# fims9000/SYNT_ISIC

Measured on AMD Instinct MI355X. Metric: images/sec at 3x64x64 T=1000 (DDPM reverse-diffusion sampling), higher is better.
Workload: dtype f32

## Files before the change

synt_isic_amd/csrc/conv_plan.cpp:

```cpp
#include "conv_plan.h"
#include "poison_switch.h"

#include <algorithm>
#include <cstdio>
#include <cstdlib>

namespace sisic {

namespace {

struct Switches { bool wino_wide, wino_bf3, wino_col, ksplit, pointwise, pointwise_bf3, pointwise_ksplit, s2_bf3, pointwise_staged_ksplit; };
const Switches& switches() {
    static const Switches sw{env_on("SISIC_WINO_WIDE"), env_on("SISIC_WINO_BF16X3"), env_on("SISIC_WINO_COL"), env_on("SISIC_KSPLIT"),
                             env_on("SISIC_POINTWISE"), env_on("SISIC_POINTWISE_BF16X3"), env_on("SISIC_POINTWISE_KSPLIT"), env_on("SISIC_S2_BF16X3"),
                             env_on("SISIC_POINTWISE_STAGED_KSPLIT")};
    return sw;
}

}

bool poison_alloc() {
    static const bool on = [] { const char* e = std::getenv("SISIC_POISON_ALLOC"); return e && std::atoi(e) != 0; }();
    return on;
}

namespace {

struct DirectTiling { int cfg, ks, stride, tw, th, wn; };
constexpr DirectTiling DIRECT[] = {
#define X(id, KS, STRIDE, MT, NT, WM, WN, TW, CIC, OCC, KSP) {id, KS, STRIDE, TW, WN * NT * 32 / TW, WN},
// ... 92 lines not shown
    if (a.tile_cfg == CFG_PWB_STAGED_KSPLIT) {
        PLAN_REFUSE_UNLESS((Cin / 8) % (4 * PWB_WAVES) == 0, "conv2d(pointwise bf16x3, staged K-split): tile_cfg 37 needs a multiple of 128 input channels");
        PLAN_REFUSE_UNLESS(HW % 64 == 0, "conv2d(pointwise bf16x3, staged K-split): tile_cfg 37 needs whole 64-pixel tiles");
        PLAN_REFUSE_UNLESS(a.Cout == 64 || a.Cout == 128 || a.Cout == 256, "conv2d(pointwise bf16x3, staged K-split): tile_cfg 37 needs 64, 128 or 256 output channels");
        PLAN_REFUSE_UNLESS(a.gn_scale == nullptr, "conv2d(pointwise bf16x3, staged K-split): tile_cfg 37 has no GroupNorm prologue");
        PLAN_REFUSE_UNLESS(!a.relu, "conv2d(pointwise bf16x3, staged K-split): tile_cfg 37 has no relu");
        PLAN_REFUSE_UNLESS(a.Cout % 64 != 0 || pwbsk_lds_bytes(Cin, a.Cout) <= PWBSK_MAX_LDS, "conv2d(pointwise bf16x3, staged K-split): tile_cfg 37 needs %zu bytes of LDS", pwbsk_lds_bytes(Cin, a.Cout));
    }
    PLAN_REFUSE_UNLESS(conv_pointwise_bf3_applicable(a), "conv2d(pointwise bf16x3): shape not supported by tile_cfg 28");
    const bool ks_ok = (Cin / 8) % (4 * PWB_WAVES) == 0;
    const bool staged_ok = a.Cout / 64 >= 6 && a.Cout / 64 <= PWBS_MAX_WAVES && pwbs_lds_bytes(Cin) <= 150 * 1024;
    if (a.tile_cfg == CFG_PWB_KSPLIT) PLAN_REFUSE_UNLESS(ks_ok, "conv2d(pointwise bf16x3, K-split): tile_cfg 35 needs a multiple of 128 input channels");
    if (a.tile_cfg == CFG_PWB_STAGED) PLAN_REFUSE_UNLESS(staged_ok, "conv2d(pointwise bf16x3, staged): tile_cfg 34 needs 384 .. 768 output channels and at most %d input channels", (150 * 1024) / 392);
    if (a.tile_cfg == CFG_PWB_STAGED_KSPLIT || (a.tile_cfg == 0 && pwbsk_routed(a, ks_ok))) pl.form = PWB_FORM_STAGED_KSPLIT;
    else if (a.tile_cfg == CFG_PWB_KSPLIT || (a.tile_cfg == 0 && ks_ok && HW <= 256 && a.Cout <= 256 && switches().pointwise_ksplit)) pl.form = PWB_FORM_KSPLIT;
    else if (a.tile_cfg == CFG_PWB_STAGED || (a.tile_cfg == 0 && staged_ok && (int64_t)a.B * (HW / 64) >= 128)) pl.form = PWB_FORM_STAGED;
    else if (a.tile_cfg == CFG_PWB_64PX || (a.tile_cfg != CFG_PWB_32PX && (int64_t)a.B * (HW / 64) * (a.Cout / 64) >= 2048)) pl.form = PWB_FORM_64PX;
    else pl.form = PWB_FORM_32PX;
    pl.carries_rider = a.gn_scale == nullptr && pl.form != PWB_FORM_STAGED;
}

int plan_direct(const sisic_conv_args& a, ConvPlan& pl) {
    const Switches& sw = switches();
    int cfg = a.tile_cfg;
    SISIC_REQUIRE(!wino_cfg_row(cfg), "conv2d: tile_cfg %d needs w_winograd, ksize 3 and stride 1", cfg);
    int Ht = pl.Hout, Wt = pl.Wout;
    if (a.ksize == 7) {
        if (cfg == 0) cfg = 41;
    } else if (a.ksize == 1 && a.stride == 2) {
        if (cfg == 0) cfg = Wt >= 24 ? 31 : (Wt >= 12 ? 32 : 33);
    } else if (a.ksize == 1) {
        SISIC_REQUIRE(!a.upsample, "conv2d: 1x1 with upsample");
        const bool pwb_forced = (cfg >= CFG_PWB && cfg <= CFG_PWB_64PX) || cfg == CFG_PWB_STAGED || cfg == CFG_PWB_KSPLIT || cfg == CFG_PWB_STAGED_KSPLIT;
        if (pwb_forced || (cfg == 0 && sw.pointwise_bf3 && conv_pointwise_bf3_applicable(a))) {
// ... 84 lines not shown
```

synt_isic_amd/csrc/conv_plan.h:

```cpp
#pragma once

#include "common.h"

namespace sisic {

enum ConvCfg : int {
    CFG_AUTO = 0, CFG_POINTWISE = 20, CFG_PWB = 28, CFG_PWB_32PX = 29, CFG_PWB_64PX = 30, CFG_PWB_STAGED = 34, CFG_PWB_KSPLIT = 35,
    CFG_S2_BF3 = 36, CFG_PWB_STAGED_KSPLIT = 37, CFG_SMALL_32ROWS = 50, CFG_SMALL_8ROWS = 51, CFG_SMALL_ONE_GROUP = 52,
    CFG_WINO_1IMG_8W = 60, CFG_WINO_4IMG_8W = 61, CFG_WINO_1IMG_16W = 62, CFG_WINO_4IMG_16W = 63,
    CFG_WINO_1IMG_8W_STAG = 64, CFG_WINO_4IMG_8W_STAG = 65, CFG_WINO_1IMG_16W_STAG = 66, CFG_WINO_4IMG_16W_STAG = 67,
    CFG_WINO_WIDE128 = 68, CFG_WINO_WIDE64 = 69, CFG_WINO_COL128 = 70, CFG_WINO_COL64 = 71, CFG_WINO_SECOND128 = 72, CFG_WINO_SECOND64 = 73,
    CFG_WINO_BF3 = 74, CFG_WINO_LATENCY128 = 78, CFG_WINO_LATENCY64 = 79, CFG_KSPLIT8_FIRST = 90, CFG_KSPLIT8_PAIR = 91, CFG_KSPLIT8_BF3 = 92,
};

#define SISIC_DIRECT_TILINGS(X) \
    X(1, 3, 1, 2, 2, 1, 4, 64, 8, 2, 1)  X(2, 3, 1, 2, 2, 1, 4, 32, 8, 2, 1)  X(3, 3, 1, 2, 2, 1, 4, 16, 8, 2, 1) \
    X(4, 3, 1, 1, 1, 2, 2, 8, 8, 2, 1)  X(5, 3, 1, 2, 1, 1, 4, 16, 8, 2, 1)  X(6, 3, 1, 2, 1, 1, 4, 64, 8, 2, 1) \
    X(7, 3, 1, 2, 1, 1, 4, 32, 8, 2, 1)  X(8, 3, 1, 1, 2, 2, 4, 32, 8, 4, 1)  X(9, 3, 1, 1, 2, 2, 4, 16, 8, 4, 1) \
    X(10, 3, 1, 1, 2, 2, 4, 32, 8, 2, 1)  X(14, 3, 1, 1, 1, 2, 4, 16, 8, 4, 1)  X(15, 3, 1, 1, 1, 2, 4, 8, 8, 4, 1) \
    X(16, 3, 1, 1, 1, 2, 2, 8, 16, 2, 2)  X(17, 3, 1, 1, 1, 2, 2, 8, 8, 2, 2)  X(11, 3, 2, 2, 1, 1, 4, 32, 8, 2, 1) \
    X(12, 3, 2, 2, 1, 1, 4, 16, 8, 2, 1)  X(13, 3, 2, 1, 1, 2, 2, 8, 8, 2, 1)  X(18, 3, 2, 1, 1, 2, 2, 8, 16, 2, 2) \
    X(19, 3, 2, 1, 1, 2, 2, 8, 8, 2, 2)  X(21, 1, 1, 2, 2, 1, 4, 256, 16, 2, 1)  X(22, 1, 1, 1, 1, 2, 2, 64, 16, 2, 1) \
    X(23, 1, 1, 2, 1, 1, 4, 128, 16, 2, 1)  X(24, 1, 1, 1, 2, 2, 4, 256, 32, 4, 1)  X(25, 1, 1, 1, 1, 2, 4, 128, 32, 4, 1) \
    X(26, 1, 1, 1, 2, 2, 4, 256, 16, 4, 1)  X(27, 1, 1, 1, 1, 2, 4, 128, 16, 4, 1)  X(31, 1, 2, 2, 1, 1, 4, 32, 16, 2, 1) \
    X(32, 1, 2, 2, 1, 1, 4, 16, 16, 2, 1)  X(33, 1, 2, 1, 1, 2, 2, 8, 16, 2, 1)  X(41, 7, 2, 2, 1, 1, 4, 32, 2, 2, 1) \
    X(42, 7, 2, 2, 1, 1, 4, 32, 4, 2, 1)

enum ConvKernel { CK_SMALLCOUT, CK_DIRECT, CK_POINTWISE, CK_POINTWISE_BF3, CK_S2_BF3, CK_WINO_FIRST, CK_WINO_SECOND, CK_WINO_THIRD, CK_WINO_BF3 };
enum PwbForm { PWB_FORM_KSPLIT, PWB_FORM_STAGED, PWB_FORM_64PX, PWB_FORM_32PX, PWB_FORM_STAGED_KSPLIT };
enum ReduceForm { REDUCE_ANY, REDUCE_64PX };

enum WinoGeometry { WG_FIRST, WG_SECOND, WG_BF3 };
struct WinoCfg {
    int cfg;
    WinoGeometry geom;
    int imgs, waves;
    bool stagger;
    int col;
    int ksplit;
    int tile_h, tile_w;
    int profile_slot;
};
const WinoCfg* wino_cfg_row(int cfg);

constexpr int CS_TW = 32, CS_CIC = 2;
constexpr int PWB_WAVES = 4;
constexpr int PWBS_MAX_WAVES = 12;
inline size_t pwbs_lds_bytes(int Cin) { return (size_t)(Cin / 8) * 2 * 64 * 24 + 8 * (size_t)Cin; }
constexpr int PWBSK_MAX_WAVES = 16, PWBSK_CAP = 8;
constexpr size_t PWBSK_MAX_LDS = 128 * 1024;
inline size_t pwbsk_lds_bytes(int Cin, int Cout) {
    const int nl = Cin / 8 / PWB_WAVES;
    const size_t operands = (size_t)PWB_WAVES * (nl < PWBSK_CAP ? nl : PWBSK_CAP) * 2 * 64 * 24, partials = (size_t)PWB_WAVES * (Cout / 64) * 32 * 64 * 4;
    return operands > partials ? operands : partials;
}

struct ConvPlan {
    ConvKernel kernel;
    int cfg;
    int form;
    int Hout, Wout, stats_slots;
    bool finalizes, carries_rider;
    int ksplit;
// ... 11 lines not shown
```

synt_isic_amd/csrc/conv_pointwise_bf3.hip:

```cpp
#include <cstdlib>
#include <type_traits>

#include "conv_plan.h"
#include "gn_finalize.h"

namespace sisic {

typedef float pwb_f32x16 __attribute__((ext_vector_type(16)));
typedef short pwb_bf16x8 __attribute__((ext_vector_type(8)));
typedef unsigned pwb_u4 __attribute__((ext_vector_type(4)));
typedef unsigned pwb_u2 __attribute__((ext_vector_type(2)));
typedef float pwb_f2 __attribute__((ext_vector_type(2)));
typedef float pwb_f4 __attribute__((ext_vector_type(4)));

struct PwbParams {
    const float* in0;
    const float* in1;
    int c0, c1, B, HW;
    const float* wb;
    int n_co64;
    const float* bias;
    int Cout;
    const float* gn_scale;
    const float* gn_shift;
    const float* chan_bias;
    int chan_bias_stride;
    const float* residual;
    int relu;
    float* out;
    float* stats;
    int n_px, n_co_items, nitems, nwg, nchunks;
    int n_rider_wg;
    GnFinJob rider;
};


__device__ __forceinline__ float pwb_half_wave_sum(float v) {
    v += __int_as_float(__builtin_amdgcn_update_dpp(0, __float_as_int(v), 0xB1, 0xf, 0xf, true));
    v += __int_as_float(__builtin_amdgcn_update_dpp(0, __float_as_int(v), 0x4E, 0xf, 0xf, true));
    v += __int_as_float(__builtin_amdgcn_update_dpp(0, __float_as_int(v), 0x141, 0xf, 0xf, true));
    v += __int_as_float(__builtin_amdgcn_update_dpp(0, __float_as_int(v), 0x140, 0xf, 0xf, true));
    return v + __shfl_xor(v, 16);
}
__device__ __forceinline__ float pwb_row16_sum(float v) {
    v += __int_as_float(__builtin_amdgcn_update_dpp(0, __float_as_int(v), 0xB1, 0xf, 0xf, true));
    v += __int_as_float(__builtin_amdgcn_update_dpp(0, __float_as_int(v), 0x4E, 0xf, 0xf, true));
    v += __int_as_float(__builtin_amdgcn_update_dpp(0, __float_as_int(v), 0x141, 0xf, 0xf, true));
    v += __int_as_float(__builtin_amdgcn_update_dpp(0, __float_as_int(v), 0x140, 0xf, 0xf, true));
// ... 404 lines not shown
        for (int i = 0; i < XD; ++i) {
            if (c + i < nl) {
                const Tup t = make(c + i, xr[i]);
                if (c + i + XD < nl) load_x(cb + c + i + XD, xr[i]);
                if ((i & 1) == 0) {
                    mm(t, ua, ul);
                    if (c + i + 2 < nl) load_f(cb + c + i + 2, ua, ul);
                } else {
                    mm(t, ub, um);
                    if (c + i + 2 < nl) load_f(cb + c + i + 2, ub, um);
                }
            }
        }
    }

#pragma unroll
    for (int x = 0; x < CB; ++x)
#pragma unroll
        for (int r = 0; r < 16; ++r) P_lds[((wave_u * 2 + x) * 16 + r) * 64 + lane] = acc[x][r];
    __syncthreads();
    const int x = wave_u >> 1, rb = 8 * (wave_u & 1);
    const __amdgpu_buffer_rsrc_t rso = __builtin_amdgcn_make_buffer_rsrc(p.out + (size_t)b * p.Cout * HW, 0, -1, 0x00020000);
    const __amdgpu_buffer_rsrc_t rsr = __builtin_amdgcn_make_buffer_rsrc(
        const_cast<float*>(p.residual ? p.residual + (size_t)b * p.Cout * HW : p.out), 0, -1, 0x00020000);
    const unsigned o_voff = 4u * (unsigned)((4 * half) * HW + px0 + l31);
    const int slots = HW / 32;
    float add[8], res[8];
#pragma unroll
    for (int rr = 0; rr < 8; ++rr) {
        const int r = rb + rr;
        const int cs = co0 + 32 * x + 8 * (r >> 2) + (r & 3);
        const int col = cs + 4 * half;
        add[rr] = 0.0f;
        if (p.bias) add[rr] += p.bias[col];
        if (p.chan_bias) add[rr] += p.chan_bias[(size_t)b * p.chan_bias_stride + col];
        res[rr] = 0.0f;
        if (p.residual) res[rr] = __builtin_bit_cast(float, __builtin_amdgcn_raw_buffer_load_b32(rsr, o_voff, 4u * (unsigned)(cs * HW), 0));
    }
#pragma unroll
    for (int rr = 0; rr < 8; ++rr) {
        const int r = rb + rr;
        const int cs = co0 + 32 * x + 8 * (r >> 2) + (r & 3);
        float part[PWB_WAVES];
#pragma unroll
        for (int k = 0; k < PWB_WAVES; ++k) part[k] = P_lds[((k * 2 + x) * 16 + r) * 64 + lane];
        float v = ((part[0] + part[1]) + part[2]) + part[3];
        v = v + add[rr] + res[rr];
        if (p.relu) v = fmaxf(v, 0.0f);
        __builtin_amdgcn_raw_buffer_store_b32(__float_as_uint(v), rso, o_voff, 4u * (unsigned)(cs * HW), 0);
        if (p.stats) {
            const int co = cs + 4 * half;
            const float s1 = pwb_half_wave_sum(v);
            const float d = v - s1 * (1.0f / 32.0f);
            float dd;
            asm volatile("v_mul_f32 %0, %1, %1" : "=v"(dd) : "v"(d));
            const float q = pwb_half_wave_sum(dd);
            if (l31 == 0)
                reinterpret_cast<float4*>(p.stats)[((size_t)b * p.Cout + co) * slots + px_t] = make_float4(32.0f, s1, q, 0.0f);
        }
    }
}

__device__ __forceinline__ void pwbs_load_chunk(const __amdgpu_buffer_rsrc_t rs0, const __amdgpu_buffer_rsrc_t rs1, const int c0, const int HW,
                                                const int c, const unsigned x_voff, pwb_f2 (&xr)[4]) {
    const int cc0 = 8 * c;
    if (cc0 < c0) {
        const unsigned soff = 4u * (unsigned)(cc0 * HW);
#pragma unroll
        for (int k = 0; k < 4; ++k) xr[k] = __builtin_bit_cast(pwb_f2, __builtin_amdgcn_raw_buffer_load_b64(rs0, x_voff, soff + 4u * (unsigned)(k * HW), 0));
    } else {
        const unsigned soff = 4u * (unsigned)((cc0 - c0) * HW);
#pragma unroll
        for (int k = 0; k < 4; ++k) xr[k] = __builtin_bit_cast(pwb_f2, __builtin_amdgcn_raw_buffer_load_b64(rs1, x_voff, soff + 4u * (unsigned)(k * HW), 0));
    }
}
template <int PRO>
__device__ __forceinline__ void pwbs_split_store(const pwb_f2 (&xr)[4], const float* gp, unsigned* const S_hm, unsigned* const S_lo, const int slot,
                                                 const int lane) {
    pwb_f4 g01 = {1.0f, 0.0f, 1.0f, 0.0f}, g23 = g01;
    if constexpr (PRO != 0) {
        g01 = *reinterpret_cast<const pwb_f4*>(gp);
        g23 = *reinterpret_cast<const pwb_f4*>(gp + 4);
    }
#pragma unroll
    for (int nb = 0; nb < 2; ++nb) {
        float v[4];
#pragma unroll
        for (int k = 0; k < 4; ++k) {
            float e = nb ? xr[k].y : xr[k].x;
            if constexpr (PRO != 0) {
                const float sc = k == 0 ? g01.x : (k == 1 ? g01.z : (k == 2 ? g23.x : g23.z));
                const float sh = k == 0 ? g01.y : (k == 1 ? g01.w : (k == 2 ? g23.y : g23.w));
                e = e * sc + sh;
                if constexpr (PRO == 2) e = pwb_silu(e);
            }
            v[k] = e;
        }
        unsigned hi[2], mid[2], lo[2];
#pragma unroll
        for (int q = 0; q < 2; ++q) {
            const float v0 = v[2 * q], v1 = v[2 * q + 1];
            const unsigned h0 = __float_as_uint(v0) & 0xffff0000u, h1 = __float_as_uint(v1) & 0xffff0000u;
            const float r0 = v0 - __uint_as_float(h0), r1 = v1 - __uint_as_float(h1);
            const unsigned m0 = __float_as_uint(r0) & 0xffff0000u, m1 = __float_as_uint(r1) & 0xffff0000u;
            const float l0 = r0 - __uint_as_float(m0), l1 = r1 - __uint_as_float(m1);
            hi[q] = __builtin_amdgcn_perm(h1, h0, 0x07060302u);
            mid[q] = __builtin_amdgcn_perm(m1, m0, 0x07060302u);
            lo[q] = __builtin_amdgcn_perm(__float_as_uint(l1), __float_as_uint(l0), 0x07060302u);
        }
        *reinterpret_cast<pwb_u4*>(S_hm + ((size_t)(slot * 2 + nb) * 64 + lane) * 4) = pwb_u4{hi[0], hi[1], mid[0], mid[1]};
        *reinterpret_cast<pwb_u2*>(S_lo + ((size_t)(slot * 2 + nb) * 64 + lane) * 2) = pwb_u2{lo[0], lo[1]};
    }
}
__device__ __forceinline__ void pwbs_read_b(const unsigned* const S_hm, const unsigned* const S_lo, const int slot, const int nb, const int lane,
                                            pwb_u4& hm, pwb_u4& mh, pwb_u4& lh) {
    hm = *reinterpret_cast<const pwb_u4*>(S_hm + ((size_t)(slot * 2 + nb) * 64 + lane) * 4);
    const pwb_u2 lo = *reinterpret_cast<const pwb_u2*>(S_lo + ((size_t)(slot * 2 + nb) * 64 + lane) * 2);
    mh = pwb_u4{hm.z, hm.w, hm.x, hm.y};
    lh = pwb_u4{lo.x, lo.y, hm.x, hm.y};
}

template <int PRO>
__global__ void __launch_bounds__(64 * PWBS_MAX_WAVES) conv_pwbs_kernel(const PwbParams p) {
    extern __shared__ __attribute__((aligned(16))) float smem[];
    int wg;
    {
        const int L = blockIdx.x, nwg = p.nwg;
        const int xcd = L & 7, slot = L >> 3, q = nwg >> 3, r = nwg & 7;
        wg = (xcd < r ? xcd * (q + 1) : r * (q + 1) + (xcd - r) * q) + slot;
    }
    const int tid = threadIdx.x, lane = tid & 63;
    const int wave_u = __builtin_amdgcn_readfirstlane(tid >> 6);
    const int nwaves = p.n_co_items;
    const int half = lane >> 5, l31 = lane & 31;
    int px_t = wg % p.n_px, b = wg / p.n_px;
    asm volatile("" : "+s"(px_t), "+s"(b));
    constexpr int CB = 2, NB = 2;
    const int co_i = wave_u;
    const int px0 = 64 * px_t, co0 = 64 * co_i;
    const int Cin = p.c0 + p.c1, HW = p.HW, n = p.nchunks;

    const __amdgpu_buffer_rsrc_t rs0 = __builtin_amdgcn_make_buffer_rsrc(const_cast<float*>(p.in0 + (size_t)b * p.c0 * HW), 0, -1, 0x00020000);
    const __amdgpu_buffer_rsrc_t rs1 = __builtin_amdgcn_make_buffer_rsrc(
        const_cast<float*>(p.in1 ? p.in1 + (size_t)b * p.c1 * HW : p.in0), 0, -1, 0x00020000);
    const __amdgpu_buffer_rsrc_t rsw = __builtin_amdgcn_make_buffer_rsrc(const_cast<float*>(p.wb), 0, -1, 0x00020000);
    const unsigned x_voff = 4u * (unsigned)((4 * half) * HW + px0 + NB * l31);
    const unsigned a_lane16 = 16u * (unsigned)lane, a_lane8 = 8u * (unsigned)lane;

    unsigned* const S_hm = reinterpret_cast<unsigned*>(smem);
    unsigned* const S_lo = S_hm + (size_t)n * NB * 64 * 4;
    float* const gnL = reinterpret_cast<float*>(S_lo + (size_t)n * NB * 64 * 2);
    if constexpr (PRO != 0) {
        for (int i = tid; i < Cin; i += 64 * nwaves) {
            gnL[2 * i] = p.gn_scale[(size_t)b * Cin + i];
            gnL[2 * i + 1] = p.gn_shift[(size_t)b * Cin + i];
        }
        __syncthreads();
    }
    for (int c = wave_u; c < n; c += nwaves) {
        pwb_f2 xr[4];
        pwbs_load_chunk(rs0, rs1, p.c0, HW, c, x_voff, xr);
        pwbs_split_store<PRO>(xr, gnL + 2 * (8 * c + 4 * half), S_hm, S_lo, c, lane);
    }
    __syncthreads();

    pwb_f32x16 acc[CB][NB];
#pragma unroll
    for (int x = 0; x < CB; ++x)
#pragma unroll
        for (int nb = 0; nb < NB; ++nb)
#pragma unroll
            for (int r = 0; r < 16; ++r) acc[x][nb][r] = 0.0f;
    pwb_u4 ua[CB], ub[CB];
    pwb_u2 ul[CB], um[CB];
    auto load_f = [&](int c, pwb_u4 (&fa)[CB], pwb_u2 (&fl)[CB]) {
        const unsigned s0 = 3072u * (unsigned)(c * p.n_co64 + co_i);
#pragma unroll
        for (int x = 0; x < CB; ++x) {
            fa[x] = __builtin_amdgcn_raw_buffer_load_b128(rsw, a_lane16, s0 + 1024u * (unsigned)x, 0);
            fl[x] = __builtin_amdgcn_raw_buffer_load_b64(rsw, a_lane8, s0 + 2048u + 512u * (unsigned)x, 0);
        }
    };
    auto chunk = [&](int c, const pwb_u4 (&fa)[CB], const pwb_u2 (&fl)[CB]) {
#pragma unroll
        for (int nb = 0; nb < NB; ++nb) {
            pwb_u4 hm, mh, lh;
            pwbs_read_b(S_hm, S_lo, c, nb, lane, hm, mh, lh);
#pragma unroll
            for (int x = 0; x < CB; ++x) {
                const pwb_u4 a_hl = {fa[x].x, fa[x].y, fl[x].x, fl[x].y};
                acc[x][nb] = __builtin_amdgcn_mfma_f32_32x32x16_bf16(__builtin_bit_cast(pwb_bf16x8, fa[x]), __builtin_bit_cast(pwb_bf16x8, hm), acc[x][nb], 0, 0, 0);
                acc[x][nb] = __builtin_amdgcn_mfma_f32_32x32x16_bf16(__builtin_bit_cast(pwb_bf16x8, fa[x]), __builtin_bit_cast(pwb_bf16x8, mh), acc[x][nb], 0, 0, 0);
                acc[x][nb] = __builtin_amdgcn_mfma_f32_32x32x16_bf16(__builtin_bit_cast(pwb_bf16x8, a_hl), __builtin_bit_cast(pwb_bf16x8, lh), acc[x][nb], 0, 0, 0);
            }
        }
    };
    load_f(0, ua, ul);
    if (n > 1) load_f(1, ub, um);
    {
        int c = 0;
        for (; c + 1 < n; c += 2) {
            chunk(c, ua, ul);
            if (c + 2 < n) load_f(c + 2, ua, ul);
            chunk(c + 1, ub, um);
            if (c + 3 < n) load_f(c + 3, ub, um);
        }
        if (c < n) chunk(c, ua, ul);
    }

    const __amdgpu_buffer_rsrc_t rso = __builtin_amdgcn_make_buffer_rsrc(p.out + (size_t)b * p.Cout * HW, 0, -1, 0x00020000);
    const __amdgpu_buffer_rsrc_t rsr = __builtin_amdgcn_make_buffer_rsrc(
        const_cast<float*>(p.residual ? p.residual + (size_t)b * p.Cout * HW : p.out), 0, -1, 0x00020000);
    const unsigned o_voff = 4u * (unsigned)((4 * half) * HW + px0 + NB * l31);
    const int slots = HW / 32;
#pragma unroll
    for (int x = 0; x < CB; ++x) {
        float add[16];
        pwb_f2 res[16];
#pragma unroll
        for (int r = 0; r < 16; ++r) {
            const int cs = co0 + 32 * x + 8 * (r >> 2) + (r & 3);
            const int col = cs + 4 * half;
            add[r] = 0.0f;
            if (p.bias) add[r] += p.bias[col];
            if (p.chan_bias) add[r] += p.chan_bias[(size_t)b * p.chan_bias_stride + col];
            res[r] = pwb_f2{0.0f, 0.0f};
            if (p.residual) res[r] = __builtin_bit_cast(pwb_f2, __builtin_amdgcn_raw_buffer_load_b64(rsr, o_voff, 4u * (unsigned)(cs * HW), 0));
        }
#pragma unroll
        for (int r = 0; r < 16; ++r) {
            const int cs = co0 + 32 * x + 8 * (r >> 2) + (r & 3);
            float vv[2];
#pragma unroll
            for (int nb = 0; nb < NB; ++nb) {
                vv[nb] = acc[x][nb][r] + add[r] + (nb ? res[r].y : res[r].x);
                if (p.relu) vv[nb] = fmaxf(vv[nb], 0.0f);
            }
            __builtin_amdgcn_raw_buffer_store_b64(pwb_u2{__float_as_uint(vv[0]), __float_as_uint(vv[1])}, rso, o_voff, 4u * (unsigned)(cs * HW), 0);
            if (p.stats) {
                const int co = cs + 4 * half;
                const float s1 = pwb_row16_sum(vv[0] + vv[1]);
                const float mean = s1 * (1.0f / 32.0f);
                const float d0 = vv[0] - mean, d1 = vv[1] - mean;
                float q0, q1;
                asm volatile("v_mul_f32 %0, %2, %2\n\tv_mul_f32 %1, %3, %3" : "=&v"(q0), "=&v"(q1) : "v"(d0), "v"(d1));
                const float q = pwb_row16_sum(q0 + q1);
                if ((l31 & 15) == 0)
                    reinterpret_cast<float4*>(p.stats)[((size_t)b * p.Cout + co) * slots + 2 * px_t + (l31 >> 4)] = make_float4(32.0f, s1, q, 0.0f);
            }
        }
    }
}

#ifndef PWBSK_VAR
#define PWBSK_VAR 0
#endif
__global__ void __launch_bounds__(64 * PWBSK_MAX_WAVES) conv_pwbsk_kernel(const PwbParams p) {
    extern __shared__ __attribute__((aligned(16))) float smem[];
    const int tid = threadIdx.x, lane = tid & 63;
    const int wave_u = __builtin_amdgcn_readfirstlane(tid >> 6);
    const int nwaves = PWB_WAVES * p.n_co_items;
    int L = blockIdx.x;
    if (L < p.n_rider_wg) {
// ... 85 lines not shown
            chunk(kq * cap + j, ua, ul);
            if (p0 + j + 2 < nl) load_f(cb + p0 + j + 2, ua, ul);
            chunk(kq * cap + j + 1, ub, um);
            if (p0 + j + 3 < nl) load_f(cb + p0 + j + 3, ub, um);
        }
#else
        acc[0][0][0] += __uint_as_float(ua[0].x ^ ub[1].y ^ ul[0].x ^ um[1].y) + __uint_as_float(S_hm[lane + 64 * kq]);
#endif
    }

    const __amdgpu_buffer_rsrc_t rso = __builtin_amdgcn_make_buffer_rsrc(p.out + (size_t)b * p.Cout * HW, 0, -1, 0x00020000);
    const __amdgpu_buffer_rsrc_t rsr = __builtin_amdgcn_make_buffer_rsrc(
        const_cast<float*>(p.residual ? p.residual + (size_t)b * p.Cout * HW : p.out), 0, -1, 0x00020000);
    const unsigned o_voff = 4u * (unsigned)((4 * half) * HW + px0 + NB * l31);
    const int slots = HW / 32;
#pragma unroll
    for (int x = 0; x < CB; ++x) {
#if (PWBSK_VAR & 4) == 0
        __syncthreads();
#pragma unroll
        for (int nb = 0; nb < NB; ++nb)
#pragma unroll
            for (int r = 0; r < 16; ++r) P_lds[((wave_u * NB + nb) * 16 + r) * 64 + lane] = acc[x][nb][r];
        __syncthreads();
#endif
        float add[4];
        pwb_f2 res[4];
#pragma unroll
        for (int rr = 0; rr < 4; ++rr) {
            const int cs = co0 + 32 * x + 8 * kq + rr;
            const int col = cs + 4 * half;
            add[rr] = 0.0f;
            if (p.bias) add[rr] += p.bias[col];
            if (p.chan_bias) add[rr] += p.chan_bias[(size_t)b * p.chan_bias_stride + col];
            res[rr] = pwb_f2{0.0f, 0.0f};
            if (p.residual) res[rr] = __builtin_bit_cast(pwb_f2, __builtin_amdgcn_raw_buffer_load_b64(rsr, o_voff, 4u * (unsigned)(cs * HW), 0));
        }
#pragma unroll
        for (int rr = 0; rr < 4; ++rr) {
            const int r = 4 * kq + rr;
            const int cs = co0 + 32 * x + 8 * kq + rr;
            float vv[NB];
#pragma unroll
            for (int nb = 0; nb < NB; ++nb) {
                float part[PWB_WAVES];
#if (PWBSK_VAR & 4) == 0
#pragma unroll
                for (int k = 0; k < PWB_WAVES; ++k) part[k] = P_lds[(((co_i * PWB_WAVES + k) * NB + nb) * 16 + r) * 64 + lane];
#else
#pragma unroll
                for (int k = 0; k < PWB_WAVES; ++k) part[k] = acc[x][nb][4 * k + rr];
#endif
// ... 41 lines not shown
    p.n_px = p.HW / 32;
    const int64_t nitems = (int64_t)p.B * p.n_px * p.n_co_items;
    SISIC_REQUIRE(nitems > 0 && nitems < (int64_t(1) << 31), "conv2d(pointwise bf16x3, K-split): grid too large");
    p.nitems = (int)nitems;
    p.nwg = p.nitems;
    SISIC_REQUIRE((int64_t)p.nwg + p.n_rider_wg < (int64_t(1) << 31), "conv2d(pointwise bf16x3, K-split): grid too large");
    const size_t lds = sizeof(float) * (size_t)(PWB_WAVES * 32 * 64 + (PRO ? 2 * Cin : 0));
    static std::atomic<uint64_t> opt{0};
    auto kern = conv_pwbk_kernel<PRO>;
    SISIC_TRY(ensure_dynamic_lds(ctx, reinterpret_cast<const void*>(kern), (int)lds, opt));
    hipLaunchKernelGGL(kern, dim3(p.n_rider_wg + p.nwg), dim3(64 * PWB_WAVES), lds, s, p);
    SISIC_HIP(hipGetLastError());
    return SISIC_OK;
}

template <int PRO>
static int launch_pwbs(sisic_ctx* ctx, PwbParams& p, int Cin, hipStream_t s) {
    p.n_co_items = p.Cout / 64;
    p.n_px = p.HW / 64;
    const int64_t nwg = (int64_t)p.B * p.n_px;
    SISIC_REQUIRE(nwg > 0 && nwg < (int64_t(1) << 31), "conv2d(pointwise bf16x3, staged): grid too large");
    p.nwg = (int)nwg;
    p.nitems = p.nwg * p.n_co_items;
    const size_t lds = pwbs_lds_bytes(Cin);
    static std::atomic<uint64_t> opt{0};
    auto kern = conv_pwbs_kernel<PRO>;
    SISIC_TRY(ensure_dynamic_lds(ctx, reinterpret_cast<const void*>(kern), (int)lds, opt));
    hipLaunchKernelGGL(kern, dim3(p.nwg), dim3(64 * p.n_co_items), lds, s, p);
    SISIC_HIP(hipGetLastError());
    return SISIC_OK;
}

bool conv_pointwise_bf3_applicable(const sisic_conv_args& a) {
    if (a.ksize != 1 || a.stride != 1 || a.upsample) return false;
    const int HW = a.Hin * a.Win, Cin = a.c0 + a.c1;
    if (HW % 64 != 0 || Cin % 8 != 0 || (a.c1 != 0 && a.c0 % 8 != 0) || a.Cout % 64 != 0) return false;
    if (((reinterpret_cast<uintptr_t>(a.in0) | reinterpret_cast<uintptr_t>(a.in1) | reinterpret_cast<uintptr_t>(a.out) |
          reinterpret_cast<uintptr_t>(a.residual)) & 7) != 0) return false;
    if (4.0 * std::max(std::max(a.c0, a.c1), a.Cout) * HW >= 4294967296.0 || 6.0 * conv_cin_pad(Cin, 1) * conv_cout_pad(a.Cout) >= 4294967296.0) return false;
    if (a.gn_scale && Cin > 1024) return false;
    return true;
}

// ... 15 lines not shown
    return SISIC_OK;
}

int launch_conv_pointwise_bf3(sisic_ctx* ctx, const sisic_conv_args& a, const ConvPlan& plan, hipStream_t s, const GnFinJob* rider) {
    PwbParams p{};
    const int Cin = a.c0 + a.c1;
    p.in0 = a.in0; p.in1 = a.in1; p.c0 = a.c0; p.c1 = a.c1; p.B = a.B; p.HW = a.Hin * a.Win;
    p.wb = a.w_packed + 2 * (size_t)conv_cin_pad(Cin, 1) * conv_cout_pad(a.Cout);
    p.n_co64 = conv_cout_pad(a.Cout) / 64;
    p.bias = a.bias; p.Cout = a.Cout;
    p.gn_scale = a.gn_scale; p.gn_shift = a.gn_shift;
    p.chan_bias = a.chan_bias; p.chan_bias_stride = a.chan_bias_stride; p.residual = a.residual; p.relu = a.relu;
    p.out = a.out; p.stats = a.stats_out;
    p.nchunks = Cin / 8;
    const int pro = a.gn_scale == nullptr ? 0 : (a.gn_silu ? 2 : 1);
    static_assert(PWB_WAVES == GNF_WAVES, "a rider workgroup runs one finalisation job per wave");
    if (rider) { p.rider = *rider; p.n_rider_wg = cdiv(rider->n_jobs, GNF_WAVES); }
    switch (plan.form) {
        case PWB_FORM_STAGED_KSPLIT:
            return launch_pwbsk(ctx, p, Cin, s, rider);
        case PWB_FORM_KSPLIT:
            return pro == 2 ? launch_pwbk<2>(ctx, p, Cin, s) : pro == 1 ? launch_pwbk<1>(ctx, p, Cin, s) : launch_pwbk<0>(ctx, p, Cin, s);
        case PWB_FORM_STAGED:
            return pro == 2 ? launch_pwbs<2>(ctx, p, Cin, s) : pro == 1 ? launch_pwbs<1>(ctx, p, Cin, s) : launch_pwbs<0>(ctx, p, Cin, s);
        case PWB_FORM_64PX:
            return pro == 2 ? launch_pwb<2, 2>(ctx, p, Cin, s) : pro == 1 ? launch_pwb<1, 2>(ctx, p, Cin, s) : launch_pwb<0, 2>(ctx, p, Cin, s);
        default:
            return pro == 2 ? launch_pwb<2, 1>(ctx, p, Cin, s) : pro == 1 ? launch_pwb<1, 1>(ctx, p, Cin, s) : launch_pwb<0, 1>(ctx, p, Cin, s);
    }
}

}
```

Measured before the change: 12.41.

## Add 32-pixel staged pointwise form, deeper weight prefetch, and optional early epilogue loads

Adds a staged pointwise bf16x3 variant that handles 32 pixels per workgroup and splits output channels across two workgroups, meant for 64-pixel feature maps with many output channels. It sits behind an environment switch. The staged kernel now prefetches weight fragments to a configurable depth and overlaps them with the input staging, batching several input chunk loads per wave. An opt-in flag hoists bias and residual loads ahead of the LDS barrier in two epilogues. With default settings only the deeper prefetch, batched staging and hoisted bias path change, at the cost of more register pressure.

```diff
diff --git a/synt_isic_amd/csrc/conv_plan.cpp b/synt_isic_amd/csrc/conv_plan.cpp
--- a/synt_isic_amd/csrc/conv_plan.cpp
+++ b/synt_isic_amd/csrc/conv_plan.cpp
@@ -9,11 +9,11 @@
 
 namespace {
 
-struct Switches { bool wino_wide, wino_bf3, wino_col, ksplit, pointwise, pointwise_bf3, pointwise_ksplit, s2_bf3, pointwise_staged_ksplit; };
+struct Switches { bool wino_wide, wino_bf3, wino_col, ksplit, pointwise, pointwise_bf3, pointwise_ksplit, s2_bf3, pointwise_staged_ksplit, pointwise_staged32; };
 const Switches& switches() {
     static const Switches sw{env_on("SISIC_WINO_WIDE"), env_on("SISIC_WINO_BF16X3"), env_on("SISIC_WINO_COL"), env_on("SISIC_KSPLIT"),
                              env_on("SISIC_POINTWISE"), env_on("SISIC_POINTWISE_BF16X3"), env_on("SISIC_POINTWISE_KSPLIT"), env_on("SISIC_S2_BF16X3"),
-                             env_on("SISIC_POINTWISE_STAGED_KSPLIT")};
+                             env_on("SISIC_POINTWISE_STAGED_KSPLIT"), env_on("SISIC_POINTWISE_STAGED32")};
     return sw;
 }
 
@@ -136,10 +136,12 @@
     if (a.tile_cfg == CFG_PWB_STAGED) PLAN_REFUSE_UNLESS(staged_ok, "conv2d(pointwise bf16x3, staged): tile_cfg 34 needs 384 .. 768 output channels and at most %d input channels", (150 * 1024) / 392);
     if (a.tile_cfg == CFG_PWB_STAGED_KSPLIT || (a.tile_cfg == 0 && pwbsk_routed(a, ks_ok))) pl.form = PWB_FORM_STAGED_KSPLIT;
     else if (a.tile_cfg == CFG_PWB_KSPLIT || (a.tile_cfg == 0 && ks_ok && HW <= 256 && a.Cout <= 256 && switches().pointwise_ksplit)) pl.form = PWB_FORM_KSPLIT;
+    else if (a.tile_cfg == 0 && switches().pointwise_staged32 && HW == 64 && a.Cout >= 384 && a.Cout / 64 <= PWBS_MAX_WAVES && pwbs_lds_bytes(Cin, 1) <= 150 * 1024)
+        pl.form = PWB_FORM_STAGED_32PX;
     else if (a.tile_cfg == CFG_PWB_STAGED || (a.tile_cfg == 0 && staged_ok && (int64_t)a.B * (HW / 64) >= 128)) pl.form = PWB_FORM_STAGED;
     else if (a.tile_cfg == CFG_PWB_64PX || (a.tile_cfg != CFG_PWB_32PX && (int64_t)a.B * (HW / 64) * (a.Cout / 64) >= 2048)) pl.form = PWB_FORM_64PX;
     else pl.form = PWB_FORM_32PX;
-    pl.carries_rider = a.gn_scale == nullptr && pl.form != PWB_FORM_STAGED;
+    pl.carries_rider = a.gn_scale == nullptr && pl.form != PWB_FORM_STAGED && pl.form != PWB_FORM_STAGED_32PX;
 }
 
 int plan_direct(const sisic_conv_args& a, ConvPlan& pl) {
diff --git a/synt_isic_amd/csrc/conv_plan.h b/synt_isic_amd/csrc/conv_plan.h
--- a/synt_isic_amd/csrc/conv_plan.h
+++ b/synt_isic_amd/csrc/conv_plan.h
@@ -27,7 +27,7 @@
     X(42, 7, 2, 2, 1, 1, 4, 32, 4, 2, 1)
 
 enum ConvKernel { CK_SMALLCOUT, CK_DIRECT, CK_POINTWISE, CK_POINTWISE_BF3, CK_S2_BF3, CK_WINO_FIRST, CK_WINO_SECOND, CK_WINO_THIRD, CK_WINO_BF3 };
-enum PwbForm { PWB_FORM_KSPLIT, PWB_FORM_STAGED, PWB_FORM_64PX, PWB_FORM_32PX, PWB_FORM_STAGED_KSPLIT };
+enum PwbForm { PWB_FORM_KSPLIT, PWB_FORM_STAGED, PWB_FORM_64PX, PWB_FORM_32PX, PWB_FORM_STAGED_KSPLIT, PWB_FORM_STAGED_32PX };
 enum ReduceForm { REDUCE_ANY, REDUCE_64PX };
 
 enum WinoGeometry { WG_FIRST, WG_SECOND, WG_BF3 };
@@ -46,7 +46,7 @@
 constexpr int CS_TW = 32, CS_CIC = 2;
 constexpr int PWB_WAVES = 4;
 constexpr int PWBS_MAX_WAVES = 12;
-inline size_t pwbs_lds_bytes(int Cin) { return (size_t)(Cin / 8) * 2 * 64 * 24 + 8 * (size_t)Cin; }
+inline size_t pwbs_lds_bytes(int Cin, int nb = 2) { return (size_t)(Cin / 8) * nb * 64 * 24 + 8 * (size_t)Cin; }
 constexpr int PWBSK_MAX_WAVES = 16, PWBSK_CAP = 8;
 constexpr size_t PWBSK_MAX_LDS = 128 * 1024;
 inline size_t pwbsk_lds_bytes(int Cin, int Cout) {
diff --git a/synt_isic_amd/csrc/conv_pointwise_bf3.hip b/synt_isic_amd/csrc/conv_pointwise_bf3.hip
--- a/synt_isic_amd/csrc/conv_pointwise_bf3.hip
+++ b/synt_isic_amd/csrc/conv_pointwise_bf3.hip
@@ -32,6 +32,8 @@
     int n_px, n_co_items, nitems, nwg, nchunks;
     int n_rider_wg;
     GnFinJob rider;
+    int co_split;
+    int early_epilogue;
 };
 
 
@@ -466,28 +468,37 @@
         }
     }
 
-#pragma unroll
-    for (int x = 0; x < CB; ++x)
-#pragma unroll
-        for (int r = 0; r < 16; ++r) P_lds[((wave_u * 2 + x) * 16 + r) * 64 + lane] = acc[x][r];
-    __syncthreads();
     const int x = wave_u >> 1, rb = 8 * (wave_u & 1);
     const __amdgpu_buffer_rsrc_t rso = __builtin_amdgcn_make_buffer_rsrc(p.out + (size_t)b * p.Cout * HW, 0, -1, 0x00020000);
     const __amdgpu_buffer_rsrc_t rsr = __builtin_amdgcn_make_buffer_rsrc(
         const_cast<float*>(p.residual ? p.residual + (size_t)b * p.Cout * HW : p.out), 0, -1, 0x00020000);
     const unsigned o_voff = 4u * (unsigned)((4 * half) * HW + px0 + l31);
     const int slots = HW / 32;
-    float add[8], res[8];
+    float bv[8], cv[8], res[8], add[8];
+    auto fetch_epilogue = [&]() {
+#pragma unroll
+        for (int rr = 0; rr < 8; ++rr) {
+            const int r = rb + rr;
+            const int cs = co0 + 32 * x + 8 * (r >> 2) + (r & 3);
+            const int col = cs + 4 * half;
+            bv[rr] = cv[rr] = res[rr] = 0.0f;
+            if (p.bias) bv[rr] = p.bias[col];
+            if (p.chan_bias) cv[rr] = p.chan_bias[(size_t)b * p.chan_bias_stride + col];
+            if (p.residual) res[rr] = __builtin_bit_cast(float, __builtin_amdgcn_raw_buffer_load_b32(rsr, o_voff, 4u * (unsigned)(cs * HW), 0));
+        }
+    };
+    if (p.early_epilogue) fetch_epilogue();
+#pragma unroll
+    for (int xx = 0; xx < CB; ++xx)
+#pragma unroll
+        for (int r = 0; r < 16; ++r) P_lds[((wave_u * 2 + xx) * 16 + r) * 64 + lane] = acc[xx][r];
+    __syncthreads();
+    if (!p.early_epilogue) fetch_epilogue();
 #pragma unroll
     for (int rr = 0; rr < 8; ++rr) {
-        const int r = rb + rr;
-        const int cs = co0 + 32 * x + 8 * (r >> 2) + (r & 3);
-        const int col = cs + 4 * half;
         add[rr] = 0.0f;
-        if (p.bias) add[rr] += p.bias[col];
-        if (p.chan_bias) add[rr] += p.chan_bias[(size_t)b * p.chan_bias_stride + col];
-        res[rr] = 0.0f;
-        if (p.residual) res[rr] = __builtin_bit_cast(float, __builtin_amdgcn_raw_buffer_load_b32(rsr, o_voff, 4u * (unsigned)(cs * HW), 0));
+        if (p.bias) add[rr] += bv[rr];
+        if (p.chan_bias) add[rr] += cv[rr];
     }
 #pragma unroll
     for (int rr = 0; rr < 8; ++rr) {
@@ -513,20 +524,26 @@
     }
 }
 
+template <int NB = 2>
+__device__ __forceinline__ pwb_f2 pwbs_load_px(const __amdgpu_buffer_rsrc_t rs, const unsigned voff, const unsigned soff) {
+    if constexpr (NB == 2) return __builtin_bit_cast(pwb_f2, __builtin_amdgcn_raw_buffer_load_b64(rs, voff, soff, 0));
+    else return pwb_f2{__builtin_bit_cast(float, __builtin_amdgcn_raw_buffer_load_b32(rs, voff, soff, 0)), 0.0f};
+}
+template <int NB = 2>
 __device__ __forceinline__ void pwbs_load_chunk(const __amdgpu_buffer_rsrc_t rs0, const __amdgpu_buffer_rsrc_t rs1, const int c0, const int HW,
                                                 const int c, const unsigned x_voff, pwb_f2 (&xr)[4]) {
     const int cc0 = 8 * c;
     if (cc0 < c0) {
         const unsigned soff = 4u * (unsigned)(cc0 * HW);
 #pragma unroll
-        for (int k = 0; k < 4; ++k) xr[k] = __builtin_bit_cast(pwb_f2, __builtin_amdgcn_raw_buffer_load_b64(rs0, x_voff, soff + 4u * (unsigned)(k * HW), 0));
+        for (int k = 0; k < 4; ++k) xr[k] = pwbs_load_px<NB>(rs0, x_voff, soff + 4u * (unsigned)(k * HW));
     } else {
         const unsigned soff = 4u * (unsigned)((cc0 - c0) * HW);
 #pragma unroll
-        for (int k = 0; k < 4; ++k) xr[k] = __builtin_bit_cast(pwb_f2, __builtin_amdgcn_raw_buffer_load_b64(rs1, x_voff, soff + 4u * (unsigned)(k * HW), 0));
-    }
-}
-template <int PRO>
+        for (int k = 0; k < 4; ++k) xr[k] = pwbs_load_px<NB>(rs1, x_voff, soff + 4u * (unsigned)(k * HW));
+    }
+}
+template <int PRO, int NB = 2>
 __device__ __forceinline__ void pwbs_split_store(const pwb_f2 (&xr)[4], const float* gp, unsigned* const S_hm, unsigned* const S_lo, const int slot,
                                                  const int lane) {
     pwb_f4 g01 = {1.0f, 0.0f, 1.0f, 0.0f}, g23 = g01;
@@ -535,7 +552,7 @@
         g23 = *reinterpret_cast<const pwb_f4*>(gp + 4);
     }
 #pragma unroll
-    for (int nb = 0; nb < 2; ++nb) {
+    for (int nb = 0; nb < NB; ++nb) {
         float v[4];
 #pragma unroll
         for (int k = 0; k < 4; ++k) {
@@ -560,19 +577,29 @@
             mid[q] = __builtin_amdgcn_perm(m1, m0, 0x07060302u);
             lo[q] = __builtin_amdgcn_perm(__float_as_uint(l1), __float_as_uint(l0), 0x07060302u);
         }
-        *reinterpret_cast<pwb_u4*>(S_hm + ((size_t)(slot * 2 + nb) * 64 + lane) * 4) = pwb_u4{hi[0], hi[1], mid[0], mid[1]};
-        *reinterpret_cast<pwb_u2*>(S_lo + ((size_t)(slot * 2 + nb) * 64 + lane) * 2) = pwb_u2{lo[0], lo[1]};
-    }
-}
+        *reinterpret_cast<pwb_u4*>(S_hm + ((size_t)(slot * NB + nb) * 64 + lane) * 4) = pwb_u4{hi[0], hi[1], mid[0], mid[1]};
+        *reinterpret_cast<pwb_u2*>(S_lo + ((size_t)(slot * NB + nb) * 64 + lane) * 2) = pwb_u2{lo[0], lo[1]};
+    }
+}
+template <int NB = 2>
 __device__ __forceinline__ void pwbs_read_b(const unsigned* const S_hm, const unsigned* const S_lo, const int slot, const int nb, const int lane,
                                             pwb_u4& hm, pwb_u4& mh, pwb_u4& lh) {
-    hm = *reinterpret_cast<const pwb_u4*>(S_hm + ((size_t)(slot * 2 + nb) * 64 + lane) * 4);
-    const pwb_u2 lo = *reinterpret_cast<const pwb_u2*>(S_lo + ((size_t)(slot * 2 + nb) * 64 + lane) * 2);
+    hm = *reinterpret_cast<const pwb_u4*>(S_hm + ((size_t)(slot * NB + nb) * 64 + lane) * 4);
+    const pwb_u2 lo = *reinterpret_cast<const pwb_u2*>(S_lo + ((size_t)(slot * NB + nb) * 64 + lane) * 2);
     mh = pwb_u4{hm.z, hm.w, hm.x, hm.y};
     lh = pwb_u4{lo.x, lo.y, hm.x, hm.y};
 }
 
-template <int PRO>
+#ifndef PWBS_DEPTH_32PX
+#define PWBS_DEPTH_32PX 4
+#endif
+#ifndef PWBS_DEPTH_64PX
+#define PWBS_DEPTH_64PX 2
+#endif
+#ifndef PWBS_CO_SPLIT_32PX
+#define PWBS_CO_SPLIT_32PX 2
+#endif
+template <int PRO, int NB>
 __global__ void __launch_bounds__(64 * PWBS_MAX_WAVES) conv_pwbs_kernel(const PwbParams p) {
     extern __shared__ __attribute__((aligned(16))) float smem[];
     int wg;
@@ -583,13 +610,15 @@
     }
     const int tid = threadIdx.x, lane = tid & 63;
     const int wave_u = __builtin_amdgcn_readfirstlane(tid >> 6);
-    const int nwaves = p.n_co_items;
+    const int nwaves = p.n_co_items / p.co_split;
     const int half = lane >> 5, l31 = lane & 31;
-    int px_t = wg % p.n_px, b = wg / p.n_px;
-    asm volatile("" : "+s"(px_t), "+s"(b));
-    constexpr int CB = 2, NB = 2;
-    const int co_i = wave_u;
-    const int px0 = 64 * px_t, co0 = 64 * co_i;
+    int part = wg % p.co_split;
+    const int t = wg / p.co_split;
+    int px_t = t % p.n_px, b = t / p.n_px;
+    asm volatile("" : "+s"(px_t), "+s"(b), "+s"(part));
+    constexpr int CB = 2;
+    const int co_i = part * nwaves + wave_u;
+    const int px0 = 32 * NB * px_t, co0 = 64 * co_i;
     const int Cin = p.c0 + p.c1, HW = p.HW, n = p.nchunks;
 
     const __amdgpu_buffer_rsrc_t rs0 = __builtin_amdgcn_make_buffer_rsrc(const_cast<float*>(p.in0 + (size_t)b * p.c0 * HW), 0, -1, 0x00020000);
@@ -602,17 +631,47 @@
     unsigned* const S_hm = reinterpret_cast<unsigned*>(smem);
     unsigned* const S_lo = S_hm + (size_t)n * NB * 64 * 4;
     float* const gnL = reinterpret_cast<float*>(S_lo + (size_t)n * NB * 64 * 2);
-    if constexpr (PRO != 0) {
-        for (int i = tid; i < Cin; i += 64 * nwaves) {
-            gnL[2 * i] = p.gn_scale[(size_t)b * Cin + i];
-            gnL[2 * i + 1] = p.gn_shift[(size_t)b * Cin + i];
-        }
-        __syncthreads();
-    }
-    for (int c = wave_u; c < n; c += nwaves) {
-        pwb_f2 xr[4];
-        pwbs_load_chunk(rs0, rs1, p.c0, HW, c, x_voff, xr);
-        pwbs_split_store<PRO>(xr, gnL + 2 * (8 * c + 4 * half), S_hm, S_lo, c, lane);
+    auto fill_gn_table = [&]() {
+        if constexpr (PRO != 0) {
+            for (int i = tid; i < Cin; i += 64 * nwaves) {
+                gnL[2 * i] = p.gn_scale[(size_t)b * Cin + i];
+                gnL[2 * i + 1] = p.gn_shift[(size_t)b * Cin + i];
+            }
+            __syncthreads();
+        }
+    };
+    constexpr int D = NB == 1 ? PWBS_DEPTH_32PX : PWBS_DEPTH_64PX;
+    pwb_u4 fa[D][CB];
+    pwb_u2 fl[D][CB];
+    auto load_f = [&](int c, pwb_u4 (&ua)[CB], pwb_u2 (&ul)[CB]) {
+        const unsigned s0 = 3072u * (unsigned)(c * p.n_co64 + co_i);
+#pragma unroll
+        for (int x = 0; x < CB; ++x) {
+            ua[x] = __builtin_amdgcn_raw_buffer_load_b128(rsw, a_lane16, s0 + 1024u * (unsigned)x, 0);
+            ul[x] = __builtin_amdgcn_raw_buffer_load_b64(rsw, a_lane8, s0 + 2048u + 512u * (unsigned)x, 0);
+        }
+    };
+    {
+        constexpr int SX = NB == 1 ? 6 : 3;
+        pwb_f2 xs[SX][4];
+        auto stage_load = [&](const int cw) {
+#pragma unroll
+            for (int i = 0; i < SX; ++i)
+                if (cw + i * nwaves < n) pwbs_load_chunk<NB>(rs0, rs1, p.c0, HW, cw + i * nwaves, x_voff, xs[i]);
+        };
+#pragma unroll
+        for (int i = 0; i < D; ++i)
+            if (i < n) load_f(i, fa[i], fl[i]);
+        stage_load(wave_u);
+        fill_gn_table();
+        for (int cw = wave_u; cw < n; cw += SX * nwaves) {
+            if (cw != wave_u) stage_load(cw);
+#pragma unroll
+            for (int i = 0; i < SX; ++i) {
+                const int c = cw + i * nwaves;
+                if (c < n) pwbs_split_store<PRO, NB>(xs[i], gnL + 2 * (8 * c + 4 * half), S_hm, S_lo, c, lane);
+            }
+        }
     }
     __syncthreads();
 
@@ -623,41 +682,36 @@
         for (int nb = 0; nb < NB; ++nb)
 #pragma unroll
             for (int r = 0; r < 16; ++r) acc[x][nb][r] = 0.0f;
-    pwb_u4 ua[CB], ub[CB];
-    pwb_u2 ul[CB], um[CB];
-    auto load_f = [&](int c, pwb_u4 (&fa)[CB], pwb_u2 (&fl)[CB]) {
-        const unsigned s0 = 3072u * (unsigned)(c * p.n_co64 + co_i);
-#pragma unroll
-        for (int x = 0; x < CB; ++x) {
-            fa[x] = __builtin_amdgcn_raw_buffer_load_b128(rsw, a_lane16, s0 + 1024u * (unsigned)x, 0);
-            fl[x] = __builtin_amdgcn_raw_buffer_load_b64(rsw, a_lane8, s0 + 2048u + 512u * (unsigned)x, 0);
-        }
-    };
-    auto chunk = [&](int c, const pwb_u4 (&fa)[CB], const pwb_u2 (&fl)[CB]) {
+    float bv[CB][16];
+#pragma unroll
+    for (int x = 0; x < CB; ++x)
+#pragma unroll
+        for (int r = 0; r < 16; ++r) {
+            bv[x][r] = 0.0f;
+            if (p.bias) bv[x][r] = p.bias[co0 + 32 * x + 8 * (r >> 2) + (r & 3) + 4 * half];
+        }
+    auto chunk = [&](int c, const pwb_u4 (&ua)[CB], const pwb_u2 (&ul)[CB]) {
 #pragma unroll
         for (int nb = 0; nb < NB; ++nb) {
             pwb_u4 hm, mh, lh;
-            pwbs_read_b(S_hm, S_lo, c, nb, lane, hm, mh, lh);
+            pwbs_read_b<NB>(S_hm, S_lo, c, nb, lane, hm, mh, lh);
 #pragma unroll
             for (int x = 0; x < CB; ++x) {
-                const pwb_u4 a_hl = {fa[x].x, fa[x].y, fl[x].x, fl[x].y};
-                acc[x][nb] = __builtin_amdgcn_mfma_f32_32x32x16_bf16(__builtin_bit_cast(pwb_bf16x8, fa[x]), __builtin_bit_cast(pwb_bf16x8, hm), acc[x][nb], 0, 0, 0);
-                acc[x][nb] = __builtin_amdgcn_mfma_f32_32x32x16_bf16(__builtin_bit_cast(pwb_bf16x8, fa[x]), __builtin_bit_cast(pwb_bf16x8, mh), acc[x][nb], 0, 0, 0);
+                const pwb_u4 a_hl = {ua[x].x, ua[x].y, ul[x].x, ul[x].y};
+                acc[x][nb] = __builtin_amdgcn_mfma_f32_32x32x16_bf16(__builtin_bit_cast(pwb_bf16x8, ua[x]), __builtin_bit_cast(pwb_bf16x8, hm), acc[x][nb], 0, 0, 0);
+                acc[x][nb] = __builtin_amdgcn_mfma_f32_32x32x16_bf16(__builtin_bit_cast(pwb_bf16x8, ua[x]), __builtin_bit_cast(pwb_bf16x8, mh), acc[x][nb], 0, 0, 0);
                 acc[x][nb] = __builtin_amdgcn_mfma_f32_32x32x16_bf16(__builtin_bit_cast(pwb_bf16x8, a_hl), __builtin_bit_cast(pwb_bf16x8, lh), acc[x][nb], 0, 0, 0);
             }
         }
     };
-    load_f(0, ua, ul);
-    if (n > 1) load_f(1, ub, um);
-    {
-        int c = 0;
-        for (; c + 1 < n; c += 2) {
-            chunk(c, ua, ul);
-            if (c + 2 < n) load_f(c + 2, ua, ul);
-            chunk(c + 1, ub, um);
-            if (c + 3 < n) load_f(c + 3, ub, um);
-        }
-        if (c < n) chunk(c, ua, ul);
+    for (int c = 0; c < n; c += D) {
+#pragma unroll
+        for (int i = 0; i < D; ++i) {
+            if (c + i < n) {
+                chunk(c + i, fa[i], fl[i]);
+                if (c + i + D < n) load_f(c + i + D, fa[i], fl[i]);
+            }
+        }
     }
 
     const __amdgpu_buffer_rsrc_t rso = __builtin_amdgcn_make_buffer_rsrc(p.out + (size_t)b * p.Cout * HW, 0, -1, 0x00020000);
@@ -674,31 +728,42 @@
             const int cs = co0 + 32 * x + 8 * (r >> 2) + (r & 3);
             const int col = cs + 4 * half;
             add[r] = 0.0f;
-            if (p.bias) add[r] += p.bias[col];
+            if (p.bias) add[r] += bv[x][r];
             if (p.chan_bias) add[r] += p.chan_bias[(size_t)b * p.chan_bias_stride + col];
             res[r] = pwb_f2{0.0f, 0.0f};
-            if (p.residual) res[r] = __builtin_bit_cast(pwb_f2, __builtin_amdgcn_raw_buffer_load_b64(rsr, o_voff, 4u * (unsigned)(cs * HW), 0));
+            if (p.residual) res[r] = pwbs_load_px<NB>(rsr, o_voff, 4u * (unsigned)(cs * HW));
         }
 #pragma unroll
         for (int r = 0; r < 16; ++r) {
             const int cs = co0 + 32 * x + 8 * (r >> 2) + (r & 3);
-            float vv[2];
+            float vv[2] = {0.0f, 0.0f};
 #pragma unroll
             for (int nb = 0; nb < NB; ++nb) {
                 vv[nb] = acc[x][nb][r] + add[r] + (nb ? res[r].y : res[r].x);
                 if (p.relu) vv[nb] = fmaxf(vv[nb], 0.0f);
             }
-            __builtin_amdgcn_raw_buffer_store_b64(pwb_u2{__float_as_uint(vv[0]), __float_as_uint(vv[1])}, rso, o_voff, 4u * (unsigned)(cs * HW), 0);
+            if constexpr (NB == 2) __builtin_amdgcn_raw_buffer_store_b64(pwb_u2{__float_as_uint(vv[0]), __float_as_uint(vv[1])}, rso, o_voff, 4u * (unsigned)(cs * HW), 0);
+            else __builtin_amdgcn_raw_buffer_store_b32(__float_as_uint(vv[0]), rso, o_voff, 4u * (unsigned)(cs * HW), 0);
             if (p.stats) {
                 const int co = cs + 4 * half;
-                const float s1 = pwb_row16_sum(vv[0] + vv[1]);
-                const float mean = s1 * (1.0f / 32.0f);
-                const float d0 = vv[0] - mean, d1 = vv[1] - mean;
-                float q0, q1;
-                asm volatile("v_mul_f32 %0, %2, %2\n\tv_mul_f32 %1, %3, %3" : "=&v"(q0), "=&v"(q1) : "v"(d0), "v"(d1));
-                const float q = pwb_row16_sum(q0 + q1);
-                if ((l31 & 15) == 0)
-                    reinterpret_cast<float4*>(p.stats)[((size_t)b * p.Cout + co) * slots + 2 * px_t + (l31 >> 4)] = make_float4(32.0f, s1, q, 0.0f);
+                if constexpr (NB == 1) {
+                    const float s1 = pwb_half_wave_sum(vv[0]);
+                    const float d = vv[0] - s1 * (1.0f / 32.0f);
+                    float dd;
+                    asm volatile("v_mul_f32 %0, %1, %1" : "=v"(dd) : "v"(d));
+                    const float q = pwb_half_wave_sum(dd);
+                    if (l31 == 0)
+                        reinterpret_cast<float4*>(p.stats)[((size_t)b * p.Cout + co) * slots + px_t] = make_float4(32.0f, s1, q, 0.0f);
+                } else {
+                    const float s1 = pwb_row16_sum(vv[0] + vv[1]);
+                    const float mean = s1 * (1.0f / 32.0f);
+                    const float d0 = vv[0] - mean, d1 = vv[1] - mean;
+                    float q0, q1;
+                    asm volatile("v_mul_f32 %0, %2, %2\n\tv_mul_f32 %1, %3, %3" : "=&v"(q0), "=&v"(q1) : "v"(d0), "v"(d1));
+                    const float q = pwb_row16_sum(q0 + q1);
+                    if ((l31 & 15) == 0)
+                        reinterpret_cast<float4*>(p.stats)[((size_t)b * p.Cout + co) * slots + 2 * px_t + (l31 >> 4)] = make_float4(32.0f, s1, q, 0.0f);
+                }
             }
         }
     }
@@ -814,6 +879,30 @@
         const_cast<float*>(p.residual ? p.residual + (size_t)b * p.Cout * HW : p.out), 0, -1, 0x00020000);
     const unsigned o_voff = 4u * (unsigned)((4 * half) * HW + px0 + NB * l31);
     const int slots = HW / 32;
+    float bv[4], cv[4];
+    pwb_f2 res2[CB][4];
+    auto fetch_bias = [&](const int x) {
+#pragma unroll
+        for (int rr = 0; rr < 4; ++rr) {
+            const int col = co0 + 32 * x + 8 * kq + rr + 4 * half;
+            bv[rr] = cv[rr] = 0.0f;
+            if (p.bias) bv[rr] = p.bias[col];
+            if (p.chan_bias) cv[rr] = p.chan_bias[(size_t)b * p.chan_bias_stride + col];
+        }
+    };
+    auto fetch_residual = [&](const int x) {
+#pragma unroll
+        for (int rr = 0; rr < 4; ++rr) {
+            const int cs = co0 + 32 * x + 8 * kq + rr;
+            res2[x][rr] = pwb_f2{0.0f, 0.0f};
+            if (p.residual) res2[x][rr] = __builtin_bit_cast(pwb_f2, __builtin_amdgcn_raw_buffer_load_b64(rsr, o_voff, 4u * (unsigned)(cs * HW), 0));
+        }
+    };
+    if (p.early_epilogue) {
+        fetch_residual(0);
+        fetch_residual(1);
+        fetch_bias(0);
+    }
 #pragma unroll
     for (int x = 0; x < CB; ++x) {
 #if (PWBSK_VAR & 4) == 0
@@ -824,18 +913,19 @@
             for (int r = 0; r < 16; ++r) P_lds[((wave_u * NB + nb) * 16 + r) * 64 + lane] = acc[x][nb][r];
         __syncthreads();
 #endif
+        if (!p.early_epilogue) {
+            fetch_bias(x);
+            fetch_residual(x);
+        }
         float add[4];
-        pwb_f2 res[4];
 #pragma unroll
         for (int rr = 0; rr < 4; ++rr) {
-            const int cs = co0 + 32 * x + 8 * kq + rr;
-            const int col = cs + 4 * half;
             add[rr] = 0.0f;
-            if (p.bias) add[rr] += p.bias[col];
-            if (p.chan_bias) add[rr] += p.chan_bias[(size_t)b * p.chan_bias_stride + col];
-            res[rr] = pwb_f2{0.0f, 0.0f};
-            if (p.residual) res[rr] = __builtin_bit_cast(pwb_f2, __builtin_amdgcn_raw_buffer_load_b64(rsr, o_voff, 4u * (unsigned)(cs * HW), 0));
-        }
+            if (p.bias) add[rr] += bv[rr];
+            if (p.chan_bias) add[rr] += cv[rr];
+        }
+        if (x == 0 && p.early_epilogue) fetch_bias(1);
+        const pwb_f2 (&res)[4] = res2[x];
 #pragma unroll
         for (int rr = 0; rr < 4; ++rr) {
             const int r = 4 * kq + rr;
@@ -907,19 +997,20 @@
     return SISIC_OK;
 }
 
-template <int PRO>
+template <int PRO, int NB = 2>
 static int launch_pwbs(sisic_ctx* ctx, PwbParams& p, int Cin, hipStream_t s) {
     p.n_co_items = p.Cout / 64;
-    p.n_px = p.HW / 64;
-    const int64_t nwg = (int64_t)p.B * p.n_px;
+    p.n_px = p.HW / (32 * NB);
+    p.co_split = (NB == 1 && p.n_co_items % PWBS_CO_SPLIT_32PX == 0) ? PWBS_CO_SPLIT_32PX : 1;
+    const int64_t nwg = (int64_t)p.B * p.n_px * p.co_split;
     SISIC_REQUIRE(nwg > 0 && nwg < (int64_t(1) << 31), "conv2d(pointwise bf16x3, staged): grid too large");
     p.nwg = (int)nwg;
-    p.nitems = p.nwg * p.n_co_items;
-    const size_t lds = pwbs_lds_bytes(Cin);
+    p.nitems = p.nwg * (p.n_co_items / p.co_split);
+    const size_t lds = pwbs_lds_bytes(Cin, NB);
     static std::atomic<uint64_t> opt{0};
-    auto kern = conv_pwbs_kernel<PRO>;
+    auto kern = conv_pwbs_kernel<PRO, NB>;
     SISIC_TRY(ensure_dynamic_lds(ctx, reinterpret_cast<const void*>(kern), (int)lds, opt));
-    hipLaunchKernelGGL(kern, dim3(p.nwg), dim3(64 * p.n_co_items), lds, s, p);
+    hipLaunchKernelGGL(kern, dim3(p.nwg), dim3(64 * (p.n_co_items / p.co_split)), lds, s, p);
     SISIC_HIP(hipGetLastError());
     return SISIC_OK;
 }
@@ -965,6 +1056,8 @@
     p.out = a.out; p.stats = a.stats_out;
     p.nchunks = Cin / 8;
     const int pro = a.gn_scale == nullptr ? 0 : (a.gn_silu ? 2 : 1);
+    static const bool early = env_on("SISIC_PW_EARLY_EPILOGUE");
+    p.early_epilogue = early ? 1 : 0;
     static_assert(PWB_WAVES == GNF_WAVES, "a rider workgroup runs one finalisation job per wave");
     if (rider) { p.rider = *rider; p.n_rider_wg = cdiv(rider->n_jobs, GNF_WAVES); }
     switch (plan.form) {
@@ -974,6 +1067,8 @@
             return pro == 2 ? launch_pwbk<2>(ctx, p, Cin, s) : pro == 1 ? launch_pwbk<1>(ctx, p, Cin, s) : launch_pwbk<0>(ctx, p, Cin, s);
         case PWB_FORM_STAGED:
             return pro == 2 ? launch_pwbs<2>(ctx, p, Cin, s) : pro == 1 ? launch_pwbs<1>(ctx, p, Cin, s) : launch_pwbs<0>(ctx, p, Cin, s);
+        case PWB_FORM_STAGED_32PX:
+            return pro == 2 ? launch_pwbs<2, 1>(ctx, p, Cin, s) : pro == 1 ? launch_pwbs<1, 1>(ctx, p, Cin, s) : launch_pwbs<0, 1>(ctx, p, Cin, s);
         case PWB_FORM_64PX:
             return pro == 2 ? launch_pwb<2, 2>(ctx, p, Cin, s) : pro == 1 ? launch_pwb<1, 2>(ctx, p, Cin, s) : launch_pwb<0, 2>(ctx, p, Cin, s);
         default:
```

After: 12.45 (median of 6 runs). Within noise of the previous version (+0.3%).
